# raahii/dcvgan

Measured on AMD Instinct MI355X. Metric: videos/sec per G+D step, 16x64x64 RGB+depth, higher is better.
Workload: dtype f32

## Files before the change

dcvgan_amd/csrc/conv_mfma.hip:

```cpp
#include "dcv_common.h"

#include <algorithm>
#include <cstdlib>
#include <map>
#include <mutex>
#include <string>
#include <type_traits>
#include <vector>

namespace dcv {

thread_local char g_err[512] = {0};
std::atomic<uint64_t> g_launches{0};
thread_local char g_last_kernel[160] = {0};
#define DCV_NOTE_KERNEL(...) snprintf(g_last_kernel, sizeof(g_last_kernel), __VA_ARGS__)

typedef float f32x16 __attribute__((ext_vector_type(16)));
typedef __bf16 bf16x8 __attribute__((ext_vector_type(8)));

std::atomic<int> g_precision{0};
struct BnView {
    const float* bx; const float* gamma; const float* beta; const float* mean; const float* invstd;
    int64_t bx_sn;
    int32_t bx_sc, bx_sh, cbn, act;
// ... 997 lines not shown
#pragma unroll
        for (int t = 0; t < T; ++t) {
            const float4 w = wrow[t];
            acc[0] += w.x * xv[t];
            if (NOC > 1) acc[1] += w.y * xv[t];
            if (NOC > 2) acc[2] += w.z * xv[t];
            if (NOC > 3) acc[3] += w.w * xv[t];
        }
    }
    if (wave > 0) {
#pragma unroll
        for (int c = 0; c < NOC; ++c) red[wave - 1][c][lane] = acc[c];
    }
    __syncthreads();
    if (wave != 0) return;
#pragma unroll
    for (int w = 0; w < 3; ++w)
#pragma unroll
        for (int c = 0; c < NOC; ++c) acc[c] += red[w][c][lane];
    if (a.slab) {
        float* __restrict__ sl = a.slab + (int64_t)blockIdx.y * a.OCp * a.Mp;
#pragma unroll
        for (int c = 0; c < 4; ++c) sl[(int64_t)c * a.Mp + m] = c < NOC ? acc[c < NOC ? c : 0] : 0.f;
        return;
    }
    if (m >= a.M) return;
    float* __restrict__ yb = a.y + a.y_off + (int64_t)n * a.y_sn + (int64_t)od * a.y_sd + (int64_t)oh * a.y_sh + (int64_t)ow * a.y_sw;
#pragma unroll
    for (int c = 0; c < NOC; ++c)
        if (c < a.OC) {
            float v = acc[c];
            float* q = yb + (int64_t)c * a.y_sc;
            if (a.accumulate) v += *q;
            *q = apply_act(v, a.act, a.slope);
        }
}

__device__ __forceinline__ void xcd_plane_map(uint32_t b, uint32_t per, uint32_t nblocks, uint32_t& plane, uint32_t& rb) {
    const uint32_t full = nblocks / (8 * per) * (8 * per);
    if (b < full) {
        const uint32_t x = b & 7, k = b >> 3;
        const uint32_t g = k / per;
        plane = x + 8 * g;
        rb = k - g * per;
    } else {
        plane = b / per;
        rb = b - plane * per;
    }
}

template <int NOC, int NH, int NW, int ND, bool W32, int IW0, bool BN = false>
__global__ __launch_bounds__(256) void thin_rows_kernel(const GatherArgs a, int RC, const BnView bv = BnView()) {
    constexpr int NR = NH + 3, T = ND * NH * NW, RPB = W32 ? 8 : 4;
    __shared__ float red[3][4 * NOC][64];
    const int tid = threadIdx.x, lane = tid & 63;
    const int wave = __builtin_amdgcn_readfirstlane(tid >> 6);
    const int col = W32 ? (lane & 31) : lane;
    const uint32_t ohq = (uint32_t)a.OH / RPB;
    uint32_t plane, rblk;
    xcd_plane_map(blockIdx.x, ohq, gridDim.x, plane, rblk);
    const int oh0 = (int)rblk * RPB + (W32 ? 4 * (lane >> 5) : 0);
    const uint32_t n = plane / (uint32_t)a.OD, od = plane - n * (uint32_t)a.OD;
    const __amdgpu_buffer_rsrc_t xrs = __builtin_amdgcn_make_buffer_rsrc(const_cast<float*>(a.x + (int64_t)n * a.x_sn), 0, 0x80000000u, 0x00020000);
    uint32_t vrow[NR];
#pragma unroll
    for (int q = 0; q < NR; ++q) {
        const int ih = oh0 + a.p_ihmin + q;
        vrow[q] = (unsigned)ih < (unsigned)a.th.size ? (uint32_t)(4 * (ih * a.x_sh + col)) : 0x80000000u;
    }
    int doff[ND];
#pragma unroll
    for (int ud = 0; ud < ND; ++ud) {
        const int id = (int)od * a.td.mul + a.td.base + a.td.delta[ud];
        doff[ud] = (unsigned)id < (unsigned)a.td.size ? 4 * id * a.x_sd : -1;
    }
    int perm[T];
    {
        typedef int32_t i32x16 __attribute__((ext_vector_type(16)));
        const i32x16 sl16 = *reinterpret_cast<const i32x16*>(a.s_local);
#pragma unroll
        for (int t = 0; t < T; ++t) perm[t] = sl16[t];
    }
    float acc[4][NOC];
#pragma unroll
    for (int p = 0; p < 4; ++p)
#pragma unroll
        for (int c = 0; c < NOC; ++c) acc[p][c] = 0.f;
    typedef float f32x4 __attribute__((ext_vector_type(4)));
    [[maybe_unused]] const __amdgpu_buffer_rsrc_t bxrs = __builtin_amdgcn_make_buffer_rsrc(const_cast<float*>(BN ? bv.bx + (int64_t)n * bv.bx_sn : a.x), 0, 0x80000000u, 0x00020000);
    [[maybe_unused]] uint32_t rowok = 0;
    if constexpr (BN) {
#pragma unroll
        for (int q = 0; q < NR; ++q) rowok |= (vrow[q] != 0x80000000u) ? 1u << q : 0u;
    }
    for (int rc = wave; rc < RC; rc += 4) {
        const f32x4* __restrict__ wrow = reinterpret_cast<const f32x4*>(a.wp) + (int64_t)rc * T;
        [[maybe_unused]] const bool bnch = BN && rc < bv.cbn;
        [[maybe_unused]] float bsc = 1.f, bsh = 0.f;
        if constexpr (BN) {
            if (bnch) {
                const float is = bv.invstd[rc];
                bsc = bv.gamma[rc] * is;
                bsh = bv.beta[rc] - bv.mean[rc] * bsc;
            }
        }
#pragma unroll
        for (int ud = 0; ud < ND; ++ud) {
            if (doff[ud] < 0) continue;
            const int soff = rc * a.s_stepA + doff[ud];
            float r[NR];
            if (BN && bnch) {
#pragma unroll
                for (int q = 0; q < NR; ++q) {
                    const float v = __builtin_bit_cast(float, __builtin_amdgcn_raw_buffer_load_b32(bxrs, vrow[q], rc * (bv.bx_sc * 4), 0));
                    const float z = v * bsc + bsh;
                    const float t = bv.act == DCV_ACT_LEAKY ? (z > 0.f ? z : z * bv.slope) : z;
                    r[q] = ((rowok >> q) & 1u) ? t : 0.f;
                }
            } else {
#pragma unroll
            for (int q = 0; q < NR; ++q) r[q] = __builtin_bit_cast(float, __builtin_amdgcn_raw_buffer_load_b32(xrs, vrow[q], soff, 0));
            }
            f32x4 w[NH * NW];
#pragma unroll
            for (int t = 0; t < NH * NW; ++t) w[t] = wrow[perm[ud * NH * NW + t]];
#pragma unroll
            for (int q = 0; q < NR; ++q) {
                float v[3];
                v[1] = r[q];
                v[0] = __builtin_bit_cast(float, __builtin_amdgcn_update_dpp(0, __builtin_bit_cast(int, r[q]), 0x138, 0xf, 0xf, true));
                v[2] = __builtin_bit_cast(float, __builtin_amdgcn_update_dpp(0, __builtin_bit_cast(int, r[q]), 0x130, 0xf, 0xf, true));
                if (W32) {
                    v[0] = col == 0 ? 0.f : v[0];
                    v[2] = col == 31 ? 0.f : v[2];
                }
#pragma unroll
                for (int p = 0; p < 4; ++p) {
                    const int ra = q - p;
                    if (ra < 0 || ra >= NH) continue;
#pragma unroll
                    for (int b = 0; b < NW; ++b) {
                        const f32x4 wt = w[ra * NW + b];
                        const float xv = v[IW0 + b + 1];
                        acc[p][0] += wt[0] * xv;
                        if (NOC > 1) acc[p][1] += wt[1] * xv;
                        if (NOC > 2) acc[p][2] += wt[2] * xv;
                        if (NOC > 3) acc[p][3] += wt[3] * xv;
                    }
                }
            }
        }
    }
    if (wave > 0) {
#pragma unroll
        for (int p = 0; p < 4; ++p)
#pragma unroll
            for (int c = 0; c < NOC; ++c) red[wave - 1][p * NOC + c][lane] = acc[p][c];
    }
    __syncthreads();
    if (wave != 0) return;
    const int OC = a.OC, act = a.act, accumulate = a.accumulate;
    const float slope = a.slope;
    float* __restrict__ yb = a.y + a.y_off + (int64_t)n * a.y_sn + (int64_t)od * a.y_sd + (int64_t)col * a.y_sw;
#pragma unroll
    for (int p = 0; p < 4; ++p)
#pragma unroll
        for (int c = 0; c < NOC; ++c) {
            if (c >= OC) continue;
            float v = acc[p][c] + ((red[0][p * NOC + c][lane] + red[1][p * NOC + c][lane]) + red[2][p * NOC + c][lane]);
            float* q = yb + (int64_t)(oh0 + p) * a.y_sh + (int64_t)c * a.y_sc;
            if (accumulate) v += *q;
            *q = apply_act(v, act, slope);
        }
}

template <int NH, int NW, int ND, bool W32, int IW0>
static void launch_thin_rows(const GatherArgs& a, int OC, int RC, dim3 grid, hipStream_t s) {
    switch (OC) {
        case 1: hipLaunchKernelGGL((thin_rows_kernel<1, NH, NW, ND, W32, IW0>), grid, dim3(256), 0, s, a, RC); break;
        case 2: hipLaunchKernelGGL((thin_rows_kernel<2, NH, NW, ND, W32, IW0>), grid, dim3(256), 0, s, a, RC); break;
        case 3: hipLaunchKernelGGL((thin_rows_kernel<3, NH, NW, ND, W32, IW0>), grid, dim3(256), 0, s, a, RC); break;
        default: hipLaunchKernelGGL((thin_rows_kernel<4, NH, NW, ND, W32, IW0>), grid, dim3(256), 0, s, a, RC); break;
    }
}

template <int RC>
__global__ __launch_bounds__(256) void widen_rows_kernel(const GatherArgs a) {
    extern __shared__ float wl[];
    const int tid = threadIdx.x, lane = tid & 63;
    const int wave = __builtin_amdgcn_readfirstlane(tid >> 6);
    const uint32_t ohq = (uint32_t)a.OH >> 2;
    const uint32_t plane = blockIdx.x / ohq;
    const int oh0 = (int)(blockIdx.x - plane * ohq) * 4;
    const uint32_t n = plane / (uint32_t)a.OD, od = plane - n * (uint32_t)a.OD;
    for (int e = tid; e < RC * 9 * a.OCp; e += 256) wl[e] = a.wp[e];
    const __amdgpu_buffer_rsrc_t xrs = __builtin_amdgcn_make_buffer_rsrc(
        const_cast<float*>(a.x + (int64_t)n * a.x_sn + (int64_t)((int)od * a.td.mul + a.td.base + a.td.delta[0]) * a.x_sd), 0, 0x80000000u, 0x00020000);
    float v[RC][6][3];
#pragma unroll
    for (int q = 0; q < 6; ++q) {
        const int ih = oh0 + a.p_ihmin + q;
        const uint32_t vo = (unsigned)ih < (unsigned)a.th.size ? (uint32_t)(4 * (ih * a.x_sh + lane)) : 0x80000000u;
#pragma unroll
        for (int rc = 0; rc < RC; ++rc) {
            const float c = __builtin_bit_cast(float, __builtin_amdgcn_raw_buffer_load_b32(xrs, vo, rc * a.s_stepA, 0));
            v[rc][q][1] = c;
            v[rc][q][0] = __builtin_bit_cast(float, __builtin_amdgcn_update_dpp(0, __builtin_bit_cast(int, c), 0x138, 0xf, 0xf, true));
            v[rc][q][2] = __builtin_bit_cast(float, __builtin_amdgcn_update_dpp(0, __builtin_bit_cast(int, c), 0x130, 0xf, 0xf, true));
        }
    }
    int perm[9];
    {
        typedef int32_t i32x16 __attribute__((ext_vector_type(16)));
        const i32x16 sl16 = *reinterpret_cast<const i32x16*>(a.s_local);
#pragma unroll
        for (int t = 0; t < 9; ++t) perm[t] = sl16[t];
    }
    __syncthreads();
    const int OC = a.OC, OCp = a.OCp, act = a.act, accumulate = a.accumulate;
    const float slope = a.slope;
    float* __restrict__ yb = a.y + a.y_off + (int64_t)n * a.y_sn + (int64_t)od * a.y_sd + (int64_t)lane * a.y_sw;
    if constexpr (RC >= 3) {
    for (int oc = wave; oc < OC; oc += 4) {
        float o[4] = {0.f, 0.f, 0.f, 0.f};
#pragma unroll
        for (int rc = 0; rc < RC; ++rc)
#pragma unroll
            for (int ra = 0; ra < 3; ++ra)
#pragma unroll
                for (int b = 0; b < 3; ++b) {
                    const float w = wl[(rc * 9 + perm[ra * 3 + b]) * OCp + oc];
#pragma unroll
                    for (int p = 0; p < 4; ++p) o[p] += w * v[rc][p + ra][b];
                }
// ... 286 lines not shown
                    const int ch = mt * 32 + (r & 3) + 8 * (r >> 2) + 4 * lhi;
                    red[wave][ch][0] = t1;
                    red[wave][ch][1] = t2;
                }
            }
        }
    }
    if (MODE == 1) {
        __syncthreads();
        if (tid < 2 * cbn) {
            const int ch = tid >> 1, w = tid & 1;
            h.partial[((int64_t)blockIdx.x * cbn + ch) * 2 + w] = ((red[0][ch][w] + red[1][ch][w]) + red[2][ch][w]) + red[3][ch][w];
        }
    }
}

__global__ __launch_bounds__(256) void head_bn_finalize_kernel(const float* __restrict__ partial, int nwg, int cbn, double count, const float* __restrict__ gamma,
                                                               const float* __restrict__ invstd, float* __restrict__ dgamma, float* __restrict__ dbeta, float* __restrict__ cst) {
    __shared__ double red[2][256];
    const int c = blockIdx.x, tid = threadIdx.x;
    double a0 = 0.0, a1 = 0.0;
    for (int w = tid; w < nwg; w += 256) {
        a0 += (double)partial[((int64_t)w * cbn + c) * 2];
        a1 += (double)partial[((int64_t)w * cbn + c) * 2 + 1];
    }
    red[0][tid] = a0; red[1][tid] = a1;
    __syncthreads();
    for (int st = 128; st > 0; st >>= 1) {
        if (tid < st) { red[0][tid] += red[0][tid + st]; red[1][tid] += red[1][tid + st]; }
        __syncthreads();
    }
    if (tid == 0) {
        const double is = (double)invstd[c], sc = (double)gamma[c] * is;
        const double S1 = red[0][0], S2 = red[1][0];
        dbeta[c] = (float)S1;
        dgamma[c] = (float)(S2 * is);
        cst[2 * c] = (float)(-sc * S1 / count);
        cst[2 * c + 1] = (float)(-sc * is * is * S2 / count);
    }
}

struct QuadArgs {
    const float* s;
    float* y;
    const float* w;
    int32_t N, RC, OC, SD, SH, OD, pad0, pad1;
    int64_t s_sn, s_sc, s_sd, s_sh;
    int64_t y_sn, y_sc, y_sd, y_sh;
    int64_t w_o, w_r;
    int32_t act, accumulate;
    float slope, pad2;
};

template <int NOC, int ND>
__global__ __launch_bounds__(256) void thin_quad_kernel(const QuadArgs a) {
    __shared__ float red[3][8 * NOC][64];
    const int tid = threadIdx.x, lane = tid & 63;
    const int wave = __builtin_amdgcn_readfirstlane(tid >> 6);
    const int col = lane & 31, hw = lane >> 5;
    const uint32_t qb = (uint32_t)a.SH >> 2;
    const uint32_t plane = blockIdx.x / qb;
    const int r0 = (int)(blockIdx.x - plane * qb) * 4 + 2 * hw;
    const uint32_t n = plane / (uint32_t)a.OD, od = plane - n * (uint32_t)a.OD;
    int roff[4];
#pragma unroll
    for (int i = 0; i < 4; ++i) {
        const int rr = r0 - 1 + i;
        roff[i] = (unsigned)rr < (unsigned)a.SH ? rr * (int)a.s_sh + col : -1;
    }
    float acc[2][2][2][NOC];
#pragma unroll
    for (int q = 0; q < 2; ++q)
#pragma unroll
        for (int h = 0; h < 2; ++h)
#pragma unroll
            for (int b = 0; b < 2; ++b)
#pragma unroll
                for (int c = 0; c < NOC; ++c) acc[q][h][b][c] = 0.f;
    const float* __restrict__ sn = a.s + (int64_t)n * a.s_sn;
#pragma unroll(ND == 1 ? 4 : 1)
    for (int rc = wave; rc < a.RC; rc += 4) {
        float ctr[ND][4];
#pragma unroll
        for (int kd = 0; kd < ND; ++kd) {
            const int sd = (int)od - kd;
            const bool in = (unsigned)sd < (unsigned)a.SD;
            const float* __restrict__ pl = sn + (int64_t)rc * a.s_sc + (int64_t)(in ? sd : 0) * a.s_sd;
#pragma unroll
            for (int i = 0; i < 4; ++i) ctr[kd][i] = (in && roff[i] >= 0) ? pl[roff[i]] : 0.f;
        }
#pragma unroll
        for (int kd = 0; kd < ND; ++kd) {
            float g[4][3];
#pragma unroll
            for (int i = 0; i < 4; ++i) {
                const float v = ctr[kd][i];
                g[i][1] = v;
                float l = __builtin_bit_cast(float, __builtin_amdgcn_update_dpp(0, __builtin_bit_cast(int, v), 0x138, 0xf, 0xf, true));
                float r = __builtin_bit_cast(float, __builtin_amdgcn_update_dpp(0, __builtin_bit_cast(int, v), 0x130, 0xf, 0xf, true));
                g[i][0] = col == 0 ? 0.f : l;
                g[i][2] = col == 31 ? 0.f : r;
            }
#pragma unroll
            for (int c = 0; c < NOC; ++c) {
                if (c >= a.OC) continue;
                typedef float f32x4 __attribute__((ext_vector_type(4)));
                const f32x4* __restrict__ wq = reinterpret_cast<const f32x4*>(a.w + (int64_t)c * a.w_o + (int64_t)rc * a.w_r + kd * 16);
                const f32x4 w0 = wq[0], w1 = wq[1], w2 = wq[2], w3 = wq[3];
#pragma unroll
                for (int q = 0; q < 2; ++q) {
                    const float (&top)[3] = g[q], (&mid)[3] = g[q + 1], (&bot)[3] = g[q + 2];
                    acc[q][0][0][c] += mid[1] * w1[1] + mid[0] * w1[3] + top[1] * w3[1] + top[0] * w3[3];
                    acc[q][0][1][c] += mid[2] * w1[0] + mid[1] * w1[2] + top[2] * w3[0] + top[1] * w3[2];
                    acc[q][1][0][c] += bot[1] * w0[1] + bot[0] * w0[3] + mid[1] * w2[1] + mid[0] * w2[3];
                    acc[q][1][1][c] += bot[2] * w0[0] + bot[1] * w0[2] + mid[2] * w2[0] + mid[1] * w2[2];
                }
            }
        }
    }
    if (wave > 0) {
#pragma unroll
        for (int q = 0; q < 2; ++q)
#pragma unroll
            for (int h = 0; h < 2; ++h)
#pragma unroll
                for (int b = 0; b < 2; ++b)
#pragma unroll
                    for (int c = 0; c < NOC; ++c) red[wave - 1][((q * 2 + h) * 2 + b) * NOC + c][lane] = acc[q][h][b][c];
    }
    __syncthreads();
    if (wave != 0) return;
    const int OC = a.OC, act = a.act, accumulate = a.accumulate;
    const float slope = a.slope;
    float* __restrict__ yb = a.y + (int64_t)n * a.y_sn + (int64_t)od * a.y_sd + 2 * col;
#pragma unroll
    for (int q = 0; q < 2; ++q)
#pragma unroll
        for (int h = 0; h < 2; ++h)
#pragma unroll
            for (int c = 0; c < NOC; ++c) {
                if (c >= OC) continue;
                float v[2];
#pragma unroll
                for (int b = 0; b < 2; ++b) {
                    const int e = ((q * 2 + h) * 2 + b) * NOC + c;
                    v[b] = acc[q][h][b][c] + ((red[0][e][lane] + red[1][e][lane]) + red[2][e][lane]);
                }
                float* dst = yb + (int64_t)(2 * (r0 + q) + h) * a.y_sh + (int64_t)c * a.y_sc;
                if (accumulate) { v[0] += dst[0]; v[1] += dst[1]; }
                dst[0] = apply_act(v[0], act, slope);
                dst[1] = apply_act(v[1], act, slope);
            }
}

template <int T>
static bool launch_thin_struct(const GatherArgs& a, int OC, int RC, int rc_per_split, dim3 grid, hipStream_t s) {
    switch (OC) {
        case 1: hipLaunchKernelGGL((thin_struct_kernel<T, 1>), grid, dim3(256), 0, s, a, RC, rc_per_split); return true;
        case 2: hipLaunchKernelGGL((thin_struct_kernel<T, 2>), grid, dim3(256), 0, s, a, RC, rc_per_split); return true;
        case 3: hipLaunchKernelGGL((thin_struct_kernel<T, 3>), grid, dim3(256), 0, s, a, RC, rc_per_split); return true;
        case 4: hipLaunchKernelGGL((thin_struct_kernel<T, 4>), grid, dim3(256), 0, s, a, RC, rc_per_split); return true;
    }
    return false;
}

struct PackArgs {
    const KEntry* ktab[4];
    float* wp[4];
    int32_t K16[4];
    int32_t fmt[4];
};
__global__ void pack_weights_kernel(const float* __restrict__ w, const PackArgs pa, int OC, int OCp, int64_t ws_o) {
    const int c = blockIdx.y;
    const int64_t i = (int64_t)blockIdx.x * blockDim.x + threadIdx.x;
    if (i >= (int64_t)pa.K16[c] * OCp) return;
    const int k = (int)(i / OCp), oc = (int)(i % OCp);
    const KEntry e = pa.ktab[c][k];
    float v = 0.f;
    if (oc < OC && !(e.tapsel >> 31)) v = w[(int64_t)oc * ws_o + e.w_off];
    if (pa.fmt[c] == 2) {
        if (X6_PHASE(k >> 4)) v = -v;
        __bf16* o = reinterpret_cast<__bf16*>(pa.wp[c]);
        const __bf16 hi = (__bf16)v;
        const float r = v - (float)hi;
        const __bf16 mid = (__bf16)r;
        const __bf16 lo = (__bf16)(r - (float)mid);
        const int64_t base = (((int64_t)(k >> 4) * 6 + ((k >> 3) & 1)) * OCp + oc) * 8 + (k & 7);
        o[base] = hi; o[base + (int64_t)2 * OCp * 8] = mid; o[base + (int64_t)4 * OCp * 8] = lo;
    } else if (pa.fmt[c]) reinterpret_cast<__bf16*>(pa.wp[c])[((int64_t)(k >> 3) * OCp + oc) * 8 + (k & 7)] = (__bf16)v;
    else pa.wp[c][i] = v;
}

struct WgradArgs {
    const float* dptr;
    const float* gptr;
    float* slab;
    const KEntry* jtab;
    int32_t M, DC, J, DCp, Jp, chunk, pad0, pad1;
    FastDiv div_sp, div_hw, div_w;
    DimTaps td, th, tw;
    int64_t d_sn, g_sn;
    int32_t d_sc4, d_sd, d_sh, d_sw;
    int32_t g_sd, g_sh, g_sw, pad2;
    int32_t g_sc4, g_sd4, log2nd, pad3;
    int32_t hw_off4[16];
// ... 1611 lines not shown
    return DCV_OK;
}

static int gather_table(const GatherOp& op, const ClassPlan& cp, DevTable* tab) {
    const GatherClass& c = op.classes[cp.ci];
    const dcv_dims5& xd = op.xd;
    std::string key = device_prefix() + op.tag;
    {
        char buf[512];
        int nn = snprintf(buf, sizeof(buf), "|g%d|%d|%d|%lld|%lld|%d|%d|%lld|%lld|%lld|%lld|", (int)cp.dstep, op.RC, op.OC, (long long)op.ws_o, (long long)op.ws_r, op.KH, op.KW,
                          (long long)xd.sc, (long long)xd.sd, (long long)xd.sh, (long long)xd.sw);
        key.append(buf, nn);
        for (int d = 0; d < 3; ++d) {
            nn = snprintf(buf, sizeof(buf), "%d:", c.taps[d].n);
            key.append(buf, nn);
            for (int u = 0; u < c.taps[d].n; ++u) {
                nn = snprintf(buf, sizeof(buf), "%d,%d;", c.taps[d].delta[u], c.tap_k[d][u]);
                key.append(buf, nn);
            }
        }
    }
    return get_table(key, [&] {
        const int64_t K = (int64_t)op.RC * cp.T;
        std::vector<KEntry> host((size_t)cp.a.KIT * 16);
        size_t k = 0;
        const int ND = c.taps[0].n, NI = c.taps[1].n * c.taps[2].n;
        for (int64_t kk = 0; kk < K; ++kk) {
            int rc, ud, ui;
            if (cp.dstep) {
                ui = (int)(kk % NI);
                const int rcl = (int)(kk / NI % 4);
                ud = ND - 1 - (int)(kk / (NI * 4) % ND);
                rc = (int)(kk / ((int64_t)NI * 4 * ND)) * 4 + rcl;
            } else {
                ui = (int)(kk % NI);
                ud = (int)(kk / NI % ND);
                rc = (int)(kk / ((int64_t)NI * ND));
            }
            const int uh = ui / c.taps[2].n, uw = ui % c.taps[2].n;
            host[k++] = KEntry{(int32_t)((int64_t)rc * xd.sc + (int64_t)c.taps[0].delta[ud] * xd.sd + (int64_t)c.taps[1].delta[uh] * xd.sh + (int64_t)c.taps[2].delta[uw] * xd.sw),
                               (1u << ud) | (1u << (8 + uh)) | (1u << (16 + uw)),
                               (int32_t)(rc * op.ws_r + ((int64_t)c.tap_k[0][ud] * op.KH + c.tap_k[1][uh]) * op.KW + c.tap_k[2][uw]), 0};
        }
        for (; k < host.size(); ++k) host[k] = KEntry{0, 1u << 31, 0, 0};
        return host;
    }, tab);
}

static int launch_class(const GatherOp& op, const ClassPlan& cp, const GatherArgs& a, const TileCfg& tc, const CallOpts& o, hipStream_t stream) {
    const int OC = op.OC, RC = op.RC, OCp = a.OCp;
    switch (cp.kind) {
    case GK::RowsBn:
        DCV_NOTE_KERNEL("thin_rows_kernel (OC %d, kind %d, BatchNorm + activation of the first %d channels on load)", OC, cp.rows_kind, o.bnview->cbn);
        hipLaunchKernelGGL((thin_rows_kernel<3, 3, 3, 1, false, -1, true>), cp.grid, dim3(256), 0, stream, a, RC, *o.bnview);
        break;
    case GK::Rows:
        DCV_NOTE_KERNEL("thin_rows_kernel (OC %d, kind %d)", OC, cp.rows_kind);
        if (cp.rows_kind == 1) launch_thin_rows<3, 3, 1, false, -1>(a, OC, RC, cp.grid, stream);
        else if (cp.rows_kind == 2 && cp.rows_iw0 == -1) launch_thin_rows<2, 2, 1, true, -1>(a, OC, RC, cp.grid, stream);
        else if (cp.rows_kind == 2) launch_thin_rows<2, 2, 1, true, 0>(a, OC, RC, cp.grid, stream);
        else if (cp.rows_iw0 == -1) launch_thin_rows<2, 2, 4, true, -1>(a, OC, RC, cp.grid, stream);
        else launch_thin_rows<2, 2, 4, true, 0>(a, OC, RC, cp.grid, stream);
        break;
    case GK::HeadBn: {
        const HeadBnRequest* hb = o.headbn;
        HeadBnArgs ha;
        memset(&ha, 0, sizeof(ha));
        ha.g = a;
        ha.bx = hb->bx; ha.bdx = hb->bdx; ha.gamma = hb->gamma; ha.beta = hb->beta; ha.mean = hb->mean; ha.invstd = hb->invstd;
        ha.cst = hb->cst; ha.partial = hb->partial;
        ha.bx_sn = hb->bxd.sn; ha.bx_sc = (int32_t)hb->bxd.sc; ha.bx_sh = (int32_t)hb->bxd.sh; ha.bx_sw = (int32_t)hb->bxd.sw;
        ha.bdx_sn = hb->bdxd.sn; ha.bdx_sc = (int32_t)hb->bdxd.sc; ha.bdx_sh = (int32_t)hb->bdxd.sh; ha.bdx_sw = (int32_t)hb->bdxd.sw;
        ha.cbn = hb->cbn; ha.groups = cp.groups; ha.slope = hb->slope;
        DCV_NOTE_KERNEL("head_bn_kernel<%d> (RGB head data gradient + BatchNorm backward of %d channels)", hb->mode, hb->cbn);
        if (hb->mode == 1) hipLaunchKernelGGL((head_bn_kernel<1>), cp.grid, dim3(256), 0, stream, ha);
        else hipLaunchKernelGGL((head_bn_kernel<2>), cp.grid, dim3(256), 0, stream, ha);
        break;
    }
    case GK::WidenMfma:
        DCV_NOTE_KERNEL("widen_mfma_kernel<%d, %d>", RC, OCp / 32);
        if (OCp == 128) hipLaunchKernelGGL((widen_mfma_kernel<3, 4>), cp.grid, dim3(256), 0, stream, a, cp.groups);
        else hipLaunchKernelGGL((widen_mfma_kernel<3, 2>), cp.grid, dim3(256), 0, stream, a, cp.groups);
        break;
    case GK::WidenRows: {
        const size_t shm = (size_t)RC * 9 * OCp * sizeof(float);
        DCV_NOTE_KERNEL("widen_rows_kernel<%d>", RC);
        switch (RC) {
            case 1: hipLaunchKernelGGL(widen_rows_kernel<1>, cp.grid, dim3(256), shm, stream, a); break;
            case 2: hipLaunchKernelGGL(widen_rows_kernel<2>, cp.grid, dim3(256), shm, stream, a); break;
            case 3: hipLaunchKernelGGL(widen_rows_kernel<3>, cp.grid, dim3(256), shm, stream, a); break;
            default: hipLaunchKernelGGL(widen_rows_kernel<4>, cp.grid, dim3(256), shm, stream, a); break;
        }
        break;
    }
    default: {
        const int KS2 = cp.KS2, T = cp.T;
        DCV_NOTE_KERNEL("%s (%d x %d tile%s)", cp.kind == GK::ThinStruct ? "thin_struct_kernel" : cp.kind == GK::ThinGather ? "thin_gather_kernel" : "gather_gemm_kernel",
                        tc.bn, tc.bm, KS2 > 1 ? ", split-K" : "");
        if (cp.kind == GK::ThinStruct) {
            const int rcps = KS2 > 1 ? a.kper * 16 / T : RC;
            if (T == 4) launch_thin_struct<4>(a, OC, RC, rcps, cp.grid, stream);
            else if (T == 9) launch_thin_struct<9>(a, OC, RC, rcps, cp.grid, stream);
            else launch_thin_struct<16>(a, OC, RC, rcps, cp.grid, stream);
        } else if (cp.kind == GK::ThinGather) hipLaunchKernelGGL(thin_gather_kernel, cp.grid, dim3(256), 0, stream, a);
        else if (tc.bn == 128 && tc.bm == 64) launch_gather<2, 1, 2, 2>(a, cp.grid, stream);
        else if (tc.bn == 64 && tc.bm == 128) launch_gather<2, 1, 1, 4>(a, cp.grid, stream);
        else if (tc.bn == 128) launch_gather<2, 2, 2, 2>(a, cp.grid, stream);
// ... 583 lines not shown
    if (mode < 0 || mode > 2) return fail(DCV_EINVAL, "set_precision: 0 = fp32, 1 = bf16 MFMA products, 2 = fp32 emulated on the bf16 matrix pipe (3 x bf16 split, 6 products)");
    g_precision.store(mode);
    return DCV_OK;
}
int dcv_get_precision(void) { return g_precision.load(); }
int dcv_version(void) { return 4; }
void dcv_abi_struct_sizes(size_t out[3]) {
    if (!out) return;
    out[0] = sizeof(dcv_dims5); out[1] = sizeof(dcv_conv_geom); out[2] = sizeof(dcv_wpack);
}
int dcv_conv_effective_precision(const dcv_conv_geom* g) {
    if (g && g->mfma >= 1 && g->mfma <= 3) return g->mfma;
    return g_precision.load() + 1;
}
uint64_t dcv_launch_count(void) { return g_launches.load(); }


static bool latent_form(const dcv_conv_geom* g, const dcv_dims5* x, const dcv_dims5* y, dcv_conv_geom* g2, dcv_dims5* y2) {
    if (!g || !x || !y || !g->transposed) return false;
    const int T = g->kd * g->kh * g->kw;
    if (T <= 1 || x->d != 1 || x->h != 1 || x->w != 1 || g->sd != 1 || g->sh != 1 || g->sw != 1 || g->pd || g->ph || g->pw) return false;
    if (y->d != g->kd || y->h != g->kh || y->w != g->kw || y->c != g->cout || (int64_t)g->cout * T >= (1ll << 30)) return false;
    const int64_t sw = 1, sh = y->w, sd = (int64_t)y->h * y->w, sc = (int64_t)y->d * y->h * y->w;
    if ((y->w > 1 && y->sw != sw) || (y->h > 1 && y->sh != sh) || (y->d > 1 && y->sd != sd) || (y->c > 1 && y->sc != sc)) return false;
    *g2 = *g;
    g2->kd = g2->kh = g2->kw = 1;
    g2->cout = g->cout * T;
    *y2 = *y;
    y2->c = g->cout * T; y2->d = y2->h = y2->w = 1;
    y2->sc = 1; y2->sd = y2->sh = y2->sw = 0;
    return true;
}



static bool plan_thin_quad(const dcv_dims5& sd_, const dcv_dims5& dd, const int k[3], const int s[3], const int p[3], int act, float slope, int accumulate, QuadArgs* a) {
    if (toggles().no_quad) return false;
    const int OC = dd.c, RC = sd_.c;
    if (OC > 4 || k[1] != 4 || k[2] != 4 || s[1] != 2 || s[2] != 2 || p[1] != 1 || p[2] != 1 || s[0] != 1 || p[0] != 0 || (k[0] != 1 && k[0] != 4)) return false;
    if (sd_.w != 32 || dd.w != 64 || dd.h != 2 * sd_.h || sd_.h % 4 != 0 || sd_.sw != 1 || dd.sw != 1) return false;
    if (dd.d != sd_.d + k[0] - 1) return false;
    if ((int64_t)dd.n * dd.d * (sd_.h / 4) >= (1ll << 31) || sd_.sh * (int64_t)sd_.h >= (1ll << 30)) return false;
    memset(a, 0, sizeof(*a));
    a->N = dd.n; a->RC = RC; a->OC = OC; a->SD = sd_.d; a->SH = sd_.h; a->OD = dd.d;
    a->s_sn = sd_.sn; a->s_sc = sd_.sc; a->s_sd = sd_.sd; a->s_sh = sd_.sh;
    a->y_sn = dd.sn; a->y_sc = dd.sc; a->y_sd = dd.sd; a->y_sh = dd.sh;
    const int T = k[0] * 16;
    a->w_o = T; a->w_r = (int64_t)OC * T;
    a->act = act; a->slope = slope; a->accumulate = accumulate;
    return true;
}
static int run_thin_quad(QuadArgs a, const float* src, float* dst, const float* w, int kd, hipStream_t stream) {
    a.s = src; a.y = dst; a.w = w;
    const dim3 grid((unsigned)((int64_t)a.N * a.OD * (a.SH / 4)));
#define DCV_QUAD(NOC_)                                                                                          \
    {                                                                                                           \
        if (kd == 1) hipLaunchKernelGGL((thin_quad_kernel<NOC_, 1>), grid, dim3(256), 0, stream, a);            \
        else hipLaunchKernelGGL((thin_quad_kernel<NOC_, 4>), grid, dim3(256), 0, stream, a);                    \
    }
    switch (a.OC) {
        case 1: DCV_QUAD(1) break;
        case 2: DCV_QUAD(2) break;
        case 3: DCV_QUAD(3) break;
        default: DCV_QUAD(4) break;
    }
#undef DCV_QUAD
    DCV_NOTE_KERNEL("thin_quad_kernel<%d, %d>", a.OC, kd);
    DCV_LAUNCH_CHECK();
    return DCV_OK;
}

struct ConvCall {
    int which = 0;
    const dcv_conv_geom* g = nullptr;
    const dcv_dims5 *xd = nullptr, *yd = nullptr;
    const float* src = nullptr; const float* w = nullptr; float* dst = nullptr;
    int act = DCV_ACT_NONE, accumulate = 0; float slope = 0.f;
    bool stats = false; float* stat = nullptr; size_t stat_bytes = 0;
    const dcv_wpack* pack = nullptr;
    const float* gate = nullptr; float gate_slope = 0.f;
};
enum class ConvPath { Gather, HeadFwd, HeadDgrad, Quad };
struct ConvPlan {
    ConvPath path = ConvPath::Gather;
    dcv_conv_geom g{}; dcv_dims5 xd{}, yd{};
    GatherOp op;
    GatherPlan gp;
    QuadArgs quad;
    size_t ws_need = 0;
};

static int plan_conv(const ConvCall& c, const CallOpts& o, ConvPlan* P, bool sizes = false) {
    if (c.which != 0 && c.which != 1) return fail(DCV_EINVAL, "conv: bad dispatch");
    if (!c.g || !c.xd || !c.yd) return fail(DCV_EINVAL, "conv: null descriptor");
    const bool latent = !c.gate && latent_form(c.g, c.xd, c.yd, &P->g, &P->yd);
    if (!latent) { P->g = *c.g; P->yd = *c.yd; }
    P->xd = *c.xd;
    const dcv_conv_geom& g = P->g;
    const dcv_dims5 &xd = P->xd, &yd = P->yd;
    const int rc0 = check_geom(&g, &xd, &yd, "conv");
    if (rc0 != DCV_OK) return rc0;
    const int which = c.which;
    const int k[3] = {g.kd, g.kh, g.kw}, s[3] = {g.sd, g.sh, g.sw}, p[3] = {g.pd, g.ph, g.pw};
    const int xi[3] = {xd.d, xd.h, xd.w}, yo[3] = {yd.d, yd.h, yd.w};
    const int T = k[0] * k[1] * k[2];
    const dcv_dims5& src = which == 0 ? xd : yd;
    const dcv_dims5& dst = which == 0 ? yd : xd;
    GatherOp& op = P->op;
    op = GatherOp();
    op.x = c.src; op.xd = src; op.y = c.dst; op.yd = dst; op.w = c.w;
    op.RC = src.c; op.OC = dst.c; op.KH = k[1]; op.KW = k[2];
// ... 247 lines not shown
```

Baseline: 655.7.

## Assign independent output tiles per wave in thin conv kernels with software prefetch

For the 3-output-channel 3x3 rows kernel and selected thin quad (transposed conv) variants, each wave now computes its own output tile over all input channels instead of four waves splitting channels and reducing through shared memory. The grid shrinks by four, the LDS reduction and __syncthreads go away, and a small ring of prefetched channel rows is loaded through buffer loads with sched barriers so memory loads overlap the FMAs. The quad path also skips out-of-range depth taps and uses explicit fmaf chains. The cost is fewer blocks, a longer serial channel loop per wave, and higher register pressure.

```diff
diff --git a/dcvgan_amd/csrc/conv_mfma.hip b/dcvgan_amd/csrc/conv_mfma.hip
--- a/dcvgan_amd/csrc/conv_mfma.hip
+++ b/dcvgan_amd/csrc/conv_mfma.hip
@@ -1073,16 +1073,28 @@
 template <int NOC, int NH, int NW, int ND, bool W32, int IW0, bool BN = false>
 __global__ __launch_bounds__(256) void thin_rows_kernel(const GatherArgs a, int RC, const BnView bv = BnView()) {
     constexpr int NR = NH + 3, T = ND * NH * NW, RPB = W32 ? 8 : 4;
-    __shared__ float red[3][4 * NOC][64];
+    constexpr bool WU = NOC == 3 && NH == 3 && NW == 3 && ND == 1 && !W32;
+    constexpr int ROWS_PF = 3;
+    __shared__ float red[WU ? 1 : 3][WU ? 1 : 4 * NOC][64];
     const int tid = threadIdx.x, lane = tid & 63;
     const int wave = __builtin_amdgcn_readfirstlane(tid >> 6);
     const int col = W32 ? (lane & 31) : lane;
     const uint32_t ohq = (uint32_t)a.OH / RPB;
     uint32_t plane, rblk;
-    xcd_plane_map(blockIdx.x, ohq, gridDim.x, plane, rblk);
+    if constexpr (WU) {
+        if ((ohq & 3u) == 0) {
+            xcd_plane_map(blockIdx.x, ohq >> 2, gridDim.x, plane, rblk);
+            rblk = rblk * 4 + (uint32_t)wave;
+        } else {
+            const uint32_t unit = blockIdx.x * 4 + (uint32_t)wave;
+            if (unit >= (uint32_t)a.M >> 8) return;
+            plane = unit / ohq;
+            rblk = unit - plane * ohq;
+        }
+    } else xcd_plane_map(blockIdx.x, ohq, gridDim.x, plane, rblk);
     const int oh0 = (int)rblk * RPB + (W32 ? 4 * (lane >> 5) : 0);
     const uint32_t n = plane / (uint32_t)a.OD, od = plane - n * (uint32_t)a.OD;
-    const __amdgpu_buffer_rsrc_t xrs = __builtin_amdgcn_make_buffer_rsrc(const_cast<float*>(a.x + (int64_t)n * a.x_sn), 0, 0x80000000u, 0x00020000);
+    [[maybe_unused]] const __amdgpu_buffer_rsrc_t xrs = __builtin_amdgcn_make_buffer_rsrc(const_cast<float*>(a.x + (int64_t)n * a.x_sn), 0, 0x80000000u, 0x00020000);
     uint32_t vrow[NR];
 #pragma unroll
     for (int q = 0; q < NR; ++q) {
@@ -1114,6 +1126,78 @@
 #pragma unroll
         for (int q = 0; q < NR; ++q) rowok |= (vrow[q] != 0x80000000u) ? 1u << q : 0u;
     }
+    if constexpr (WU) {
+        float buf[ROWS_PF][NR];
+        int lrc = 0;
+        const bool inside = doff[0] >= 0;
+        auto load_ch = [&](float (&dst)[NR]) {
+            const int c = min(lrc, RC - 1);
+            const bool bn = BN && c < bv.cbn;
+            const float* base = bn ? bv.bx + (int64_t)n * bv.bx_sn : a.x + (int64_t)n * a.x_sn;
+            const int soff = bn ? c * (bv.bx_sc * 4) : c * a.s_stepA + doff[0];
+            const __amdgpu_buffer_rsrc_t rs = __builtin_amdgcn_make_buffer_rsrc(const_cast<float*>(base), 0, __builtin_amdgcn_readfirstlane(lrc < RC && inside ? 0x80000000u : 0u), 0x00020000);
+#pragma unroll
+            for (int q = 0; q < NR; ++q) dst[q] = __builtin_bit_cast(float, __builtin_amdgcn_raw_buffer_load_b32(rs, vrow[q], inside ? soff : 0, 0));
+            ++lrc;
+        };
+#pragma unroll
+        for (int j = 0; j < ROWS_PF; ++j) load_ch(buf[j]);
+        int rc = 0;
+        auto step = [&](float (&rows)[NR], bool reload) {
+            __builtin_amdgcn_sched_barrier(0);
+            const f32x4* __restrict__ wrow = reinterpret_cast<const f32x4*>(a.wp) + (int64_t)rc * T;
+            float r[NR];
+            if (BN && rc < bv.cbn) {
+                const float is = bv.invstd[rc];
+                const float bsc = bv.gamma[rc] * is;
+                const float bsh = bv.beta[rc] - bv.mean[rc] * bsc;
+#pragma unroll
+                for (int q = 0; q < NR; ++q) {
+                    const float z = rows[q] * bsc + bsh;
+                    const float t = bv.act == DCV_ACT_LEAKY ? (z > 0.f ? z : z * bv.slope) : z;
+                    r[q] = ((rowok >> q) & 1u) ? t : 0.f;
+                }
+            } else {
+#pragma unroll
+                for (int q = 0; q < NR; ++q) r[q] = rows[q];
+            }
+            f32x4 w[NH * NW];
+#pragma unroll
+            for (int t = 0; t < NH * NW; ++t) w[t] = wrow[perm[t]];
+#pragma unroll
+            for (int q = 0; q < NR; ++q) {
+                float v[3];
+                v[1] = r[q];
+                v[0] = __builtin_bit_cast(float, __builtin_amdgcn_update_dpp(0, __builtin_bit_cast(int, r[q]), 0x138, 0xf, 0xf, true));
+                v[2] = __builtin_bit_cast(float, __builtin_amdgcn_update_dpp(0, __builtin_bit_cast(int, r[q]), 0x130, 0xf, 0xf, true));
+#pragma unroll
+                for (int p = 0; p < 4; ++p) {
+                    const int ra = q - p;
+                    if (ra < 0 || ra >= NH) continue;
+#pragma unroll
+                    for (int b = 0; b < NW; ++b) {
+                        const f32x4 wt = w[ra * NW + b];
+                        const float xv = v[IW0 + b + 1];
+                        acc[p][0] += wt[0] * xv;
+                        if (NOC > 1) acc[p][1] += wt[1] * xv;
+                        if (NOC > 2) acc[p][2] += wt[2] * xv;
+                        if (NOC > 3) acc[p][3] += wt[3] * xv;
+                    }
+                }
+            }
+            ++rc;
+            __builtin_amdgcn_sched_barrier(0);
+            if (reload) load_ch(rows);
+        };
+        int t = 0;
+        for (; t + ROWS_PF <= RC; t += ROWS_PF) {
+#pragma unroll
+            for (int j = 0; j < ROWS_PF; ++j) step(buf[j], true);
+        }
+#pragma unroll
+        for (int j = 0; j < ROWS_PF - 1; ++j)
+            if (t + j < RC) step(buf[j], false);
+    } else
     for (int rc = wave; rc < RC; rc += 4) {
         const f32x4* __restrict__ wrow = reinterpret_cast<const f32x4*>(a.wp) + (int64_t)rc * T;
         [[maybe_unused]] const bool bnch = BN && rc < bv.cbn;
@@ -1172,14 +1256,16 @@
             }
         }
     }
-    if (wave > 0) {
-#pragma unroll
-        for (int p = 0; p < 4; ++p)
-#pragma unroll
-            for (int c = 0; c < NOC; ++c) red[wave - 1][p * NOC + c][lane] = acc[p][c];
-    }
-    __syncthreads();
-    if (wave != 0) return;
+    if constexpr (!WU) {
+        if (wave > 0) {
+#pragma unroll
+            for (int p = 0; p < 4; ++p)
+#pragma unroll
+                for (int c = 0; c < NOC; ++c) red[wave - 1][p * NOC + c][lane] = acc[p][c];
+        }
+        __syncthreads();
+        if (wave != 0) return;
+    }
     const int OC = a.OC, act = a.act, accumulate = a.accumulate;
     const float slope = a.slope;
     float* __restrict__ yb = a.y + a.y_off + (int64_t)n * a.y_sn + (int64_t)od * a.y_sd + (int64_t)col * a.y_sw;
@@ -1188,7 +1274,8 @@
 #pragma unroll
         for (int c = 0; c < NOC; ++c) {
             if (c >= OC) continue;
-            float v = acc[p][c] + ((red[0][p * NOC + c][lane] + red[1][p * NOC + c][lane]) + red[2][p * NOC + c][lane]);
+            float v = acc[p][c];
+            if constexpr (!WU) v += (red[0][p * NOC + c][lane] + red[1][p * NOC + c][lane]) + red[2][p * NOC + c][lane];
             float* q = yb + (int64_t)(oh0 + p) * a.y_sh + (int64_t)c * a.y_sc;
             if (accumulate) v += *q;
             *q = apply_act(v, act, slope);
@@ -1200,7 +1287,9 @@
     switch (OC) {
         case 1: hipLaunchKernelGGL((thin_rows_kernel<1, NH, NW, ND, W32, IW0>), grid, dim3(256), 0, s, a, RC); break;
         case 2: hipLaunchKernelGGL((thin_rows_kernel<2, NH, NW, ND, W32, IW0>), grid, dim3(256), 0, s, a, RC); break;
-        case 3: hipLaunchKernelGGL((thin_rows_kernel<3, NH, NW, ND, W32, IW0>), grid, dim3(256), 0, s, a, RC); break;
+        case 3:
+            hipLaunchKernelGGL((thin_rows_kernel<3, NH, NW, ND, W32, IW0>), (NH == 3 && NW == 3 && ND == 1 && !W32) ? dim3((grid.x + 3) / 4) : grid, dim3(256), 0, s, a, RC);
+            break;
         default: hipLaunchKernelGGL((thin_rows_kernel<4, NH, NW, ND, W32, IW0>), grid, dim3(256), 0, s, a, RC); break;
     }
 }
@@ -1593,49 +1682,59 @@
     float slope, pad2;
 };
 
+__host__ __device__ constexpr bool quad_wave_units(int noc, int nd) { return (noc == 3 && nd == 4) || (noc == 1 && nd == 1); }
+
 template <int NOC, int ND>
 __global__ __launch_bounds__(256) void thin_quad_kernel(const QuadArgs a) {
-    __shared__ float red[3][8 * NOC][64];
-    const int tid = threadIdx.x, lane = tid & 63;
-    const int wave = __builtin_amdgcn_readfirstlane(tid >> 6);
-    const int col = lane & 31, hw = lane >> 5;
-    const uint32_t qb = (uint32_t)a.SH >> 2;
-    const uint32_t plane = blockIdx.x / qb;
-    const int r0 = (int)(blockIdx.x - plane * qb) * 4 + 2 * hw;
-    const uint32_t n = plane / (uint32_t)a.OD, od = plane - n * (uint32_t)a.OD;
-    int roff[4];
-#pragma unroll
-    for (int i = 0; i < 4; ++i) {
-        const int rr = r0 - 1 + i;
-        roff[i] = (unsigned)rr < (unsigned)a.SH ? rr * (int)a.s_sh + col : -1;
-    }
-    float acc[2][2][2][NOC];
-#pragma unroll
-    for (int q = 0; q < 2; ++q)
-#pragma unroll
-        for (int h = 0; h < 2; ++h)
-#pragma unroll
-            for (int b = 0; b < 2; ++b)
-#pragma unroll
-                for (int c = 0; c < NOC; ++c) acc[q][h][b][c] = 0.f;
-    const float* __restrict__ sn = a.s + (int64_t)n * a.s_sn;
-#pragma unroll(ND == 1 ? 4 : 1)
-    for (int rc = wave; rc < a.RC; rc += 4) {
-        float ctr[ND][4];
-#pragma unroll
-        for (int kd = 0; kd < ND; ++kd) {
-            const int sd = (int)od - kd;
-            const bool in = (unsigned)sd < (unsigned)a.SD;
-            const float* __restrict__ pl = sn + (int64_t)rc * a.s_sc + (int64_t)(in ? sd : 0) * a.s_sd;
-#pragma unroll
-            for (int i = 0; i < 4; ++i) ctr[kd][i] = (in && roff[i] >= 0) ? pl[roff[i]] : 0.f;
-        }
-#pragma unroll
-        for (int kd = 0; kd < ND; ++kd) {
+    if constexpr (quad_wave_units(NOC, ND)) {
+        constexpr int QUAD_PF = 4;
+        const int tid = threadIdx.x, lane = tid & 63;
+        const int wave = __builtin_amdgcn_readfirstlane(tid >> 6);
+        const int col = lane & 31, hw = lane >> 5;
+        const uint32_t qb = (uint32_t)a.SH >> 2;
+        const uint32_t unit = blockIdx.x * 4 + (uint32_t)wave;
+        if (unit >= (uint32_t)a.N * (uint32_t)a.OD * qb) return;
+        const uint32_t plane = unit / qb;
+        const int r0 = (int)(unit - plane * qb) * 4 + 2 * hw;
+        const uint32_t n = plane / (uint32_t)a.OD, od = plane - n * (uint32_t)a.OD;
+        const uint32_t nrec = __builtin_amdgcn_readfirstlane(4u * ((uint32_t)(a.SH - 1) * (uint32_t)a.s_sh + 32u));
+        uint32_t voff[4];
+#pragma unroll
+        for (int i = 0; i < 4; ++i) {
+            const int rr = r0 - 1 + i;
+            voff[i] = (unsigned)rr < (unsigned)a.SH ? 4u * (uint32_t)(rr * (int)a.s_sh + col) : nrec;
+        }
+        const int kd_lo = ND == 1 ? 0 : max(0, (int)od - a.SD + 1);
+        const int nk = ND == 1 ? 1 : min(ND - 1, (int)od) - kd_lo + 1;
+        const int total = a.RC * nk;
+        float acc[2][2][2][NOC];
+#pragma unroll
+        for (int q = 0; q < 2; ++q)
+#pragma unroll
+            for (int h = 0; h < 2; ++h)
+#pragma unroll
+                for (int b = 0; b < 2; ++b)
+#pragma unroll
+                    for (int c = 0; c < NOC; ++c) acc[q][h][b][c] = 0.f;
+        const float* __restrict__ sn = a.s + (int64_t)n * a.s_sn;
+        float buf[QUAD_PF][4];
+        int lrc = 0, lkd = kd_lo;
+        auto load_step = [&](float (&dst)[4]) {
+            const float* pl = sn + (int64_t)min(lrc, a.RC - 1) * a.s_sc + (int64_t)((int)od - lkd) * a.s_sd;
+            const __amdgpu_buffer_rsrc_t rs = __builtin_amdgcn_make_buffer_rsrc(const_cast<float*>(pl), 0, __builtin_amdgcn_readfirstlane(lrc < a.RC ? nrec : 0u), 0x00020000);
+#pragma unroll
+            for (int i = 0; i < 4; ++i) dst[i] = __builtin_bit_cast(float, __builtin_amdgcn_raw_buffer_load_b32(rs, voff[i], 0, 0));
+            if (++lkd == kd_lo + nk) { lkd = kd_lo; ++lrc; }
+        };
+#pragma unroll
+        for (int j = 0; j < QUAD_PF; ++j) load_step(buf[j]);
+        int rc = 0, kd = kd_lo;
+        auto step = [&](float (&rows)[4], bool reload) {
+            __builtin_amdgcn_sched_barrier(0);
             float g[4][3];
 #pragma unroll
             for (int i = 0; i < 4; ++i) {
-                const float v = ctr[kd][i];
+                const float v = rows[i];
                 g[i][1] = v;
                 float l = __builtin_bit_cast(float, __builtin_amdgcn_update_dpp(0, __builtin_bit_cast(int, v), 0x138, 0xf, 0xf, true));
                 float r = __builtin_bit_cast(float, __builtin_amdgcn_update_dpp(0, __builtin_bit_cast(int, v), 0x130, 0xf, 0xf, true));
@@ -1644,54 +1743,148 @@
             }
 #pragma unroll
             for (int c = 0; c < NOC; ++c) {
-                if (c >= a.OC) continue;
                 typedef float f32x4 __attribute__((ext_vector_type(4)));
                 const f32x4* __restrict__ wq = reinterpret_cast<const f32x4*>(a.w + (int64_t)c * a.w_o + (int64_t)rc * a.w_r + kd * 16);
                 const f32x4 w0 = wq[0], w1 = wq[1], w2 = wq[2], w3 = wq[3];
 #pragma unroll
                 for (int q = 0; q < 2; ++q) {
                     const float (&top)[3] = g[q], (&mid)[3] = g[q + 1], (&bot)[3] = g[q + 2];
-                    acc[q][0][0][c] += mid[1] * w1[1] + mid[0] * w1[3] + top[1] * w3[1] + top[0] * w3[3];
-                    acc[q][0][1][c] += mid[2] * w1[0] + mid[1] * w1[2] + top[2] * w3[0] + top[1] * w3[2];
-                    acc[q][1][0][c] += bot[1] * w0[1] + bot[0] * w0[3] + mid[1] * w2[1] + mid[0] * w2[3];
-                    acc[q][1][1][c] += bot[2] * w0[0] + bot[1] * w0[2] + mid[2] * w2[0] + mid[1] * w2[2];
+                    float& o00 = acc[q][0][0][c];
+                    float& o01 = acc[q][0][1][c];
+                    float& o10 = acc[q][1][0][c];
+                    float& o11 = acc[q][1][1][c];
+                    o00 = fmaf(top[0], w3[3], fmaf(top[1], w3[1], fmaf(mid[0], w1[3], fmaf(mid[1], w1[1], o00))));
+                    o01 = fmaf(top[1], w3[2], fmaf(top[2], w3[0], fmaf(mid[1], w1[2], fmaf(mid[2], w1[0], o01))));
+                    o10 = fmaf(mid[0], w2[3], fmaf(mid[1], w2[1], fmaf(bot[0], w0[3], fmaf(bot[1], w0[1], o10))));
+                    o11 = fmaf(mid[1], w2[2], fmaf(mid[2], w2[0], fmaf(bot[1], w0[2], fmaf(bot[2], w0[0], o11))));
                 }
             }
-        }
-    }
-    if (wave > 0) {
+            if (++kd == kd_lo + nk) { kd = kd_lo; ++rc; }
+            __builtin_amdgcn_sched_barrier(0);
+            if (reload) load_step(rows);
+        };
+        int t = 0;
+        for (; t + QUAD_PF <= total; t += QUAD_PF) {
+#pragma unroll
+            for (int j = 0; j < QUAD_PF; ++j) step(buf[j], true);
+        }
+#pragma unroll
+        for (int j = 0; j < QUAD_PF - 1; ++j)
+            if (t + j < total) step(buf[j], false);
+        const int act = a.act, accumulate = a.accumulate;
+        const float slope = a.slope;
+        float* __restrict__ yb = a.y + (int64_t)n * a.y_sn + (int64_t)od * a.y_sd + 2 * col;
 #pragma unroll
         for (int q = 0; q < 2; ++q)
 #pragma unroll
             for (int h = 0; h < 2; ++h)
 #pragma unroll
+                for (int c = 0; c < NOC; ++c) {
+                    float v[2] = {acc[q][h][0][c], acc[q][h][1][c]};
+                    float* dst = yb + (int64_t)(2 * (r0 + q) + h) * a.y_sh + (int64_t)c * a.y_sc;
+                    if (accumulate) { v[0] += dst[0]; v[1] += dst[1]; }
+                    dst[0] = apply_act(v[0], act, slope);
+                    dst[1] = apply_act(v[1], act, slope);
+                }
+    } else {
+        __shared__ float red[3][8 * NOC][64];
+        const int tid = threadIdx.x, lane = tid & 63;
+        const int wave = __builtin_amdgcn_readfirstlane(tid >> 6);
+        const int col = lane & 31, hw = lane >> 5;
+        const uint32_t qb = (uint32_t)a.SH >> 2;
+        const uint32_t plane = blockIdx.x / qb;
+        const int r0 = (int)(blockIdx.x - plane * qb) * 4 + 2 * hw;
+        const uint32_t n = plane / (uint32_t)a.OD, od = plane - n * (uint32_t)a.OD;
+        int roff[4];
+#pragma unroll
+        for (int i = 0; i < 4; ++i) {
+            const int rr = r0 - 1 + i;
+            roff[i] = (unsigned)rr < (unsigned)a.SH ? rr * (int)a.s_sh + col : -1;
+        }
+        float acc[2][2][2][NOC];
+#pragma unroll
+        for (int q = 0; q < 2; ++q)
+#pragma unroll
+            for (int h = 0; h < 2; ++h)
+#pragma unroll
                 for (int b = 0; b < 2; ++b)
 #pragma unroll
-                    for (int c = 0; c < NOC; ++c) red[wave - 1][((q * 2 + h) * 2 + b) * NOC + c][lane] = acc[q][h][b][c];
-    }
-    __syncthreads();
-    if (wave != 0) return;
-    const int OC = a.OC, act = a.act, accumulate = a.accumulate;
-    const float slope = a.slope;
-    float* __restrict__ yb = a.y + (int64_t)n * a.y_sn + (int64_t)od * a.y_sd + 2 * col;
-#pragma unroll
-    for (int q = 0; q < 2; ++q)
-#pragma unroll
-        for (int h = 0; h < 2; ++h)
-#pragma unroll
-            for (int c = 0; c < NOC; ++c) {
-                if (c >= OC) continue;
-                float v[2];
-#pragma unroll
-                for (int b = 0; b < 2; ++b) {
-                    const int e = ((q * 2 + h) * 2 + b) * NOC + c;
-                    v[b] = acc[q][h][b][c] + ((red[0][e][lane] + red[1][e][lane]) + red[2][e][lane]);
+                    for (int c = 0; c < NOC; ++c) acc[q][h][b][c] = 0.f;
+        const float* __restrict__ sn = a.s + (int64_t)n * a.s_sn;
+#pragma unroll(ND == 1 ? 4 : 1)
+        for (int rc = wave; rc < a.RC; rc += 4) {
+            float ctr[ND][4];
+#pragma unroll
+            for (int kd = 0; kd < ND; ++kd) {
+                const int sd = (int)od - kd;
+                const bool in = (unsigned)sd < (unsigned)a.SD;
+                const float* __restrict__ pl = sn + (int64_t)rc * a.s_sc + (int64_t)(in ? sd : 0) * a.s_sd;
+#pragma unroll
+                for (int i = 0; i < 4; ++i) ctr[kd][i] = (in && roff[i] >= 0) ? pl[roff[i]] : 0.f;
+            }
+#pragma unroll
+            for (int kd = 0; kd < ND; ++kd) {
+                float g[4][3];
+#pragma unroll
+                for (int i = 0; i < 4; ++i) {
+                    const float v = ctr[kd][i];
+                    g[i][1] = v;
+                    float l = __builtin_bit_cast(float, __builtin_amdgcn_update_dpp(0, __builtin_bit_cast(int, v), 0x138, 0xf, 0xf, true));
+                    float r = __builtin_bit_cast(float, __builtin_amdgcn_update_dpp(0, __builtin_bit_cast(int, v), 0x130, 0xf, 0xf, true));
+                    g[i][0] = col == 0 ? 0.f : l;
+                    g[i][2] = col == 31 ? 0.f : r;
                 }
-                float* dst = yb + (int64_t)(2 * (r0 + q) + h) * a.y_sh + (int64_t)c * a.y_sc;
-                if (accumulate) { v[0] += dst[0]; v[1] += dst[1]; }
-                dst[0] = apply_act(v[0], act, slope);
-                dst[1] = apply_act(v[1], act, slope);
-            }
+#pragma unroll
+                for (int c = 0; c < NOC; ++c) {
+                    if (c >= a.OC) continue;
+                    typedef float f32x4 __attribute__((ext_vector_type(4)));
+                    const f32x4* __restrict__ wq = reinterpret_cast<const f32x4*>(a.w + (int64_t)c * a.w_o + (int64_t)rc * a.w_r + kd * 16);
+                    const f32x4 w0 = wq[0], w1 = wq[1], w2 = wq[2], w3 = wq[3];
+#pragma unroll
+                    for (int q = 0; q < 2; ++q) {
+                        const float (&top)[3] = g[q], (&mid)[3] = g[q + 1], (&bot)[3] = g[q + 2];
+                        acc[q][0][0][c] += mid[1] * w1[1] + mid[0] * w1[3] + top[1] * w3[1] + top[0] * w3[3];
+                        acc[q][0][1][c] += mid[2] * w1[0] + mid[1] * w1[2] + top[2] * w3[0] + top[1] * w3[2];
+                        acc[q][1][0][c] += bot[1] * w0[1] + bot[0] * w0[3] + mid[1] * w2[1] + mid[0] * w2[3];
+                        acc[q][1][1][c] += bot[2] * w0[0] + bot[1] * w0[2] + mid[2] * w2[0] + mid[1] * w2[2];
+                    }
+                }
+            }
+        }
+        if (wave > 0) {
+#pragma unroll
+            for (int q = 0; q < 2; ++q)
+#pragma unroll
+                for (int h = 0; h < 2; ++h)
+#pragma unroll
+                    for (int b = 0; b < 2; ++b)
+#pragma unroll
+                        for (int c = 0; c < NOC; ++c) red[wave - 1][((q * 2 + h) * 2 + b) * NOC + c][lane] = acc[q][h][b][c];
+        }
+        __syncthreads();
+        if (wave != 0) return;
+        const int OC = a.OC, act = a.act, accumulate = a.accumulate;
+        const float slope = a.slope;
+        float* __restrict__ yb = a.y + (int64_t)n * a.y_sn + (int64_t)od * a.y_sd + 2 * col;
+#pragma unroll
+        for (int q = 0; q < 2; ++q)
+#pragma unroll
+            for (int h = 0; h < 2; ++h)
+#pragma unroll
+                for (int c = 0; c < NOC; ++c) {
+                    if (c >= OC) continue;
+                    float v[2];
+#pragma unroll
+                    for (int b = 0; b < 2; ++b) {
+                        const int e = ((q * 2 + h) * 2 + b) * NOC + c;
+                        v[b] = acc[q][h][b][c] + ((red[0][e][lane] + red[1][e][lane]) + red[2][e][lane]);
+                    }
+                    float* dst = yb + (int64_t)(2 * (r0 + q) + h) * a.y_sh + (int64_t)c * a.y_sc;
+                    if (accumulate) { v[0] += dst[0]; v[1] += dst[1]; }
+                    dst[0] = apply_act(v[0], act, slope);
+                    dst[1] = apply_act(v[1], act, slope);
+                }
+    }
 }
 
 template <int T>
@@ -3409,7 +3602,7 @@
     switch (cp.kind) {
     case GK::RowsBn:
         DCV_NOTE_KERNEL("thin_rows_kernel (OC %d, kind %d, BatchNorm + activation of the first %d channels on load)", OC, cp.rows_kind, o.bnview->cbn);
-        hipLaunchKernelGGL((thin_rows_kernel<3, 3, 3, 1, false, -1, true>), cp.grid, dim3(256), 0, stream, a, RC, *o.bnview);
+        hipLaunchKernelGGL((thin_rows_kernel<3, 3, 3, 1, false, -1, true>), dim3((cp.grid.x + 3) / 4), dim3(256), 0, stream, a, RC, *o.bnview);
         break;
     case GK::Rows:
         DCV_NOTE_KERNEL("thin_rows_kernel (OC %d, kind %d)", OC, cp.rows_kind);
@@ -4099,11 +4292,11 @@
 }
 static int run_thin_quad(QuadArgs a, const float* src, float* dst, const float* w, int kd, hipStream_t stream) {
     a.s = src; a.y = dst; a.w = w;
-    const dim3 grid((unsigned)((int64_t)a.N * a.OD * (a.SH / 4)));
+    const int64_t units = (int64_t)a.N * a.OD * (a.SH / 4);
 #define DCV_QUAD(NOC_)                                                                                          \
     {                                                                                                           \
-        if (kd == 1) hipLaunchKernelGGL((thin_quad_kernel<NOC_, 1>), grid, dim3(256), 0, stream, a);            \
-        else hipLaunchKernelGGL((thin_quad_kernel<NOC_, 4>), grid, dim3(256), 0, stream, a);                    \
+        if (kd == 1) hipLaunchKernelGGL((thin_quad_kernel<NOC_, 1>), dim3((unsigned)(quad_wave_units(NOC_, 1) ? (units + 3) / 4 : units)), dim3(256), 0, stream, a); \
+        else hipLaunchKernelGGL((thin_quad_kernel<NOC_, 4>), dim3((unsigned)(quad_wave_units(NOC_, 4) ? (units + 3) / 4 : units)), dim3(256), 0, stream, a);         \
     }
     switch (a.OC) {
         case 1: DCV_QUAD(1) break;
```

New measurement: 654.0. Within noise of the previous version (-0.3%).
